# OliBomby/Mapperatorinator

Hardware: NVIDIA H100
Metric: event tokens/sec end-to-end (mel+T5+DiT) (higher is better)
Workload: dtype f32

## Files before the change

### mapperatorinator_b200/csrc/engine_dit.cu

```cuda
#include <algorithm>
#include <cmath>
#include <cstring>
#include <map>
#include <tuple>
#include <unordered_map>
#include <vector>

#include "../../include/mapperatorinator_b200.h"
#include "common.cuh"
#include "kernels.h"

using namespace mb200;

namespace {

struct DevBufD {
    void* p = nullptr; size_t bytes = 0;
    int ensure(size_t need) {
        if (need <= bytes) return 0;
        if (p) cudaFree(p);
        p = nullptr; bytes = 0;
        MB_CUDA_CHECK(cudaMalloc(&p, need));
        bytes = need;
        return 0;
// ... 224 lines not shown
    dd->t0_w = W("t_embedder.mlp.0.weight"); dd->t0_b = W("t_embedder.mlp.0.bias"); dd->t2_w = W("t_embedder.mlp.2.weight"); dd->t2_b = W("t_embedder.mlp.2.bias");
    dd->y0_w = W("y_embedder.class_embedding.0.weight"); dd->y0_b = W("y_embedder.class_embedding.0.bias");
    dd->y2_w = W("y_embedder.class_embedding.2.weight"); dd->y2_b = W("y_embedder.class_embedding.2.bias");
    dd->fada_w = W("final_layer.adaLN_modulation.1.weight"); dd->fada_b = W("final_layer.adaLN_modulation.1.bias");
    dd->flin_w = W("final_layer.linear.weight"); dd->flin_b = W("final_layer.linear.bias");
    for (int i = 0; i < c.depth; ++i) {
        const std::string p = "blocks." + std::to_string(i) + ".";
        dd->blocks.push_back(BlockW{W(p + "attn.in_proj_weight"), W(p + "attn.in_proj_bias"), W(p + "attn.out_proj.weight"), W(p + "attn.out_proj.bias"),
                                    W(p + "mlp.fc1.weight"), W(p + "mlp.fc1.bias"), W(p + "mlp.fc2.weight"), W(p + "mlp.fc2.bias"),
                                    W(p + "adaLN_modulation.1.weight"), W(p + "adaLN_modulation.1.bias")});
    }
    {
        int dev = 0;
        cudaGetDevice(&dev);
        cudaDeviceGetAttribute(&dd->gemm.num_sms, cudaDevAttrMultiProcessorCount, dev);
    }
    for (const auto& n : names)
        if (n.find("weight") != std::string::npos && sizes.at(n) >= (size_t)64 * 32) MB_TRY(dd->gemm.register_weight(W(n), (long long)sizes.at(n)));
    MB_CUDA_CHECK(cudaDeviceSynchronize());
    dd->pos_freqs = W("__pos_freqs"); dd->t_freqs = W("__t_freqs");
    MB_REQUIRE(dd->host_w.at("context_embedder.mlp.0.weight").size() == (size_t)d * (c.in_channels * c.pos_freq_dim + c.context_size),
               "context_embedder shape mismatch");
    {
        const size_t R = (size_t)std::max(2, c.max_batch) * c.max_seq_len;
        const size_t K0 = (size_t)c.in_channels * c.pos_freq_dim + c.context_size;
        MB_TRY(dd->gemm.reserve((size_t)64 << 20, R * std::max((size_t)d * c.mlp_ratio, K0) * 8 + 1024));
        dd->gemm.frozen = true;
        MB_TRY(dd->attn.reserve(attn_tc_workspace_bytes(std::max(2, c.max_batch), c.heads, c.max_seq_len, c.max_seq_len)));
        dd->attn.frozen = true;
    }
    dd->host_w.clear();
    dd->finalized = true;
    return 0;
}

namespace {

GemmParams gb(const float* A, long long lda, const float* W, long long ldw, float* C, long long ldc, const float* bias, int M, int N, int K) {
    GemmParams g{};
    g.A = plain_map(A, lda); g.W = W; g.ldw = ldw; g.C = plain_map(C, ldc); g.bias = bias; g.act = ACT_NONE; g.alpha = 1.f;
    g.gate = nullptr; g.gate_ld = 0; g.gate_rpb = 1; g.R = RowMap{nullptr, 0, 0, 0}; g.M = M; g.N = N; g.K = K;
    return g;
}

int ln_mod(const float* x, float* y, const float* shift, const float* scale, long long mod_ld, int T, int rows, int d, cudaStream_t st) {
    LayerNormParams p{};
    p.x = x; p.ldx = d; p.y = y; p.ldy = d; p.weight = nullptr; p.bias = nullptr; p.shift = shift; p.scale = scale; p.mod_ld = mod_ld;
    p.rows_per_batch = T; p.rows = rows; p.dim = d; p.eps = 1e-6f;
    return launch_layernorm(p, st);
// ... 280 lines not shown
```

### mapperatorinator_b200/csrc/engine_model.cu

```cuda
#include <algorithm>
#include <cstring>
#include <functional>
#include <map>
#include <tuple>
#include <unordered_map>
#include <vector>

#include "../../include/mapperatorinator_b200.h"
#include "common.cuh"
#include "kernels.h"

using namespace mb200;

namespace {

struct DevBuf {
    void* p = nullptr;
    size_t bytes = 0;
    int ensure(size_t need, bool zero = false) {
        if (need <= bytes) return 0;
        if (p) cudaFree(p);
        p = nullptr; bytes = 0;
        MB_CUDA_CHECK(cudaMalloc(&p, need));
        bytes = need;
// ... 258 lines not shown
        if (cross) {
            l.ln2_w = base + o.v[6]; l.ln2_b = base + o.v[7]; l.wq_c = base + o.v[8]; l.bq_c = base + o.v[9];
            l.wkv_c = base + o.v[10]; l.bkv_c = base + o.v[11]; l.wo_c = base + o.v[12]; l.bo_c = base + o.v[13];
        }
        l.ln3_w = base + o.v[14]; l.ln3_b = base + o.v[15]; l.fc1_w = base + o.v[16]; l.fc1_b = base + o.v[17];
        l.fc2_w = base + o.v[18]; l.fc2_b = base + o.v[19];
        return l;
    };
    for (auto& o : eo) m->enc.push_back(fill(o, false));
    for (auto& o : dof) m->dec.push_back(fill(o, true));
    m->host_w.clear();
    {
        const long long dd = (long long)d * d;
        auto reg = [&](const float* w, long long n) -> int { return m->gemm.register_weight(w, n); };
        MB_TRY(reg(m->emb_w, (long long)d * c.mel.n_mels));
        MB_TRY(reg(m->conv1_w, 3 * dd)); MB_TRY(reg(m->conv2_w, 3 * dd));
        for (const auto& l : m->enc) {
            MB_TRY(reg(l.wqkv, 3 * dd)); MB_TRY(reg(l.wo, dd));
            MB_TRY(reg(l.fc1_w, (long long)f * d)); MB_TRY(reg(l.fc2_w, (long long)f * d));
        }
        for (const auto& l : m->dec) MB_TRY(reg(l.wkv_c, 2 * dd));
        MB_CUDA_CHECK(cudaDeviceSynchronize());
        const size_t chunk = (size_t)std::min(std::max(1, c.max_windows), 16);
        const size_t a_floats = std::max({chunk * (size_t)(c.src_seq_len / 2) * f, chunk * (size_t)(c.src_seq_len + 2) * d,
                                          chunk * (size_t)c.src_seq_len * c.mel.n_mels});
        m->gemm.num_sms = std::max(1, m->num_sms_phys);
        MB_TRY(m->gemm.reserve((size_t)64 << 20, a_floats * 8 + 1024));
        m->gemm.frozen = true;
        MB_TRY(m->attn.reserve(attn_tc_workspace_bytes((int)chunk, c.heads, c.src_seq_len / 2, c.src_seq_len / 2)));
        m->attn.frozen = true;
    }

    m->max_rows = std::max(1, c.max_batch);
    MB_TRY(m->cross_kv.ensure((size_t)c.decoder_layers * m->cross_layer_stride() * sizeof(float)));
    MB_TRY(m->self_kv.ensure((size_t)c.decoder_layers * m->self_layer_stride() * sizeof(float)));
    MB_TRY(m->g_state.ensure(sizeof(GenState) + (size_t)m->max_rows * sizeof(RowState)));
    MB_TRY(m->g_cfg.ensure((size_t)m->max_rows * sizeof(SampleConfig)));
    MB_TRY(m->g_vflags.ensure((size_t)m->max_rows * c.vocab_size_in));
    MB_TRY(m->g_ids.ensure((size_t)m->max_rows * c.tgt_seq_len * sizeof(long long)));
    MB_TRY(m->g_prefill_ids.ensure((size_t)m->max_rows * c.tgt_seq_len * sizeof(long long)));
    MB_TRY(m->g_keyvalid.ensure((size_t)m->max_rows * c.tgt_seq_len));
    MB_TRY(m->g_leftpad.ensure(m->max_rows * sizeof(int)));
    MB_TRY(m->g_rowslot.ensure((size_t)3 * m->max_rows * sizeof(int)));
    MB_TRY(m->g_finished.ensure(m->max_rows));
    {
        const size_t tgt = (size_t)m->max_rows * c.tgt_seq_len;
        m->h_stage_bytes = tgt * 8 * 2 + tgt + (size_t)2 * m->max_rows * 4 + c.vocab_size_in + sizeof(GenState) + sizeof(SampleConfig) + 8 * 16;
        MB_CUDA_CHECK(cudaMallocHost(&m->h_stage, m->h_stage_bytes));
        MB_CUDA_CHECK(cudaEventCreateWithFlags(&m->stage_ev, cudaEventDisableTiming));
    }
// ... 1160 lines not shown
```

### mapperatorinator_b200/csrc/gemm.cu

```cuda
#include <algorithm>
#include <cstdlib>
#include "common.cuh"
#include "kernels.h"

namespace mb200 {

namespace {

constexpr int BM = 128, BN = 128, BK = 16, PAD = 4;

template <int MH>
__global__ void __launch_bounds__(256, 2) gemm_f32_kernel(GemmParams p) {
    constexpr int TM = 64 * MH;
    __shared__ __align__(16) float As[2][BK][TM + PAD];
    __shared__ __align__(16) float Bs[2][BK][BN + PAD];

    const int tid = threadIdx.x;
    const int tx = tid & 15, ty = tid >> 4;
    const long long m0 = (long long)blockIdx.y * TM;
    const int n0 = blockIdx.x * BN;

    const int lrow = tid >> 2;
    const int lk = (tid & 3) * 4;
    const float* a_ptr[2];
// ... 100 lines not shown
                if (rrow) v += rrow[nn];
                crow[nn] = v;
            }
        }
    }
}

__global__ void __launch_bounds__(256) gemm_splitk_reduce_kernel(GemmParams p) {
    const long long idx = (long long)blockIdx.x * 256 + threadIdx.x;
    if (idx >= (long long)p.M * p.N) return;
    const long long m = idx / p.N;
    const int n = (int)(idx - m * p.N);
    float v = p.splitk_ws[m * p.N + n];
    for (int z = 1; z < p.splitk; ++z) v += p.splitk_ws[((long long)z * p.M + m) * p.N + n];
    if (p.bias) v += __ldg(p.bias + n);
    v = apply_act(v, p.act) * p.alpha;
    if (p.gate) v *= __ldg(p.gate + ((p.m_base + m) / p.gate_rpb) * p.gate_ld + n);
    if (p.R.ptr) v += p.R.row(p.m_base + m)[n];
    p.C.row(p.m_base + m)[n] = v;
}

}

int GemmCtx::reserve(size_t splitk_need, size_t a_split_need) {
    auto grow = [&](float*& ptr, size_t& have, size_t need) -> int {
        if (need <= have) return 0;
        MB_REQUIRE(!frozen, "GEMM scratch is referenced by a captured CUDA graph and cannot grow (reserve the largest shape before capturing)");
        if (ptr) MB_CUDA_CHECK(cudaFree(ptr));
        ptr = nullptr; have = 0;
        MB_CUDA_CHECK(cudaMalloc(&ptr, need));
        have = need;
        return 0;
    };
    int s = grow(splitk_ws, splitk_bytes, splitk_need);
    if (s) return s;
    s = grow(a_split, a_split_bytes, a_split_need);
    if (s) return s;
    if (!tc_err) { MB_CUDA_CHECK(cudaMalloc(&tc_err, 4)); MB_CUDA_CHECK(cudaMemset(tc_err, 0, 4)); }
    return 0;
}

int GemmCtx::error() {
    if (!tc_err) return 0;
    int h = 0;
    cudaMemcpy(&h, tc_err, 4, cudaMemcpyDeviceToHost);
    return h;
}

void GemmCtx::destroy() {
    for (auto& kv : mirrors) cudaFree(const_cast<float*>(kv.second.hi));
    mirrors.clear();
    if (splitk_ws) cudaFree(splitk_ws);
    if (a_split) cudaFree(a_split);
    if (tc_err) cudaFree(tc_err);
    splitk_ws = a_split = nullptr; tc_err = nullptr; splitk_bytes = a_split_bytes = 0; frozen = false;
}

GemmCtx* default_gemm_ctx() {
    static GemmCtx ctx;
    static bool init = false;
    if (!init) {
        int dev = 0;
        cudaGetDevice(&dev);
        cudaDeviceGetAttribute(&ctx.num_sms, cudaDevAttrMultiProcessorCount, dev);
        init = true;
    }
    return &ctx;
}

int gemm_splits_simt(int N, int K, int num_sms, int* k_per_split) {
    const int tiles_n = (N + BN - 1) / BN;
    int splits = 1;
    if (tiles_n * 2 <= num_sms && K >= 64) splits = std::max(1, std::min((num_sms + tiles_n - 1) / tiles_n, K / 32));
    const int kps = ((K + splits - 1) / splits + BK - 1) / BK * BK;
    splits = (K + kps - 1) / kps;
    *k_per_split = kps;
    return splits;
}
// ... 8 lines not shown
int launch_gemm(const GemmParams& p, cudaStream_t stream, GemmCtx* ctx) {
    MB_REQUIRE(ctx != nullptr, "GEMM needs its engine's scratch context");
    MB_REQUIRE(p.K % 4 == 0, "GEMM K must be a multiple of 4 (float4 loads)");
    MB_REQUIRE(p.A.ld % 4 == 0 && p.ldw % 4 == 0, "GEMM operand row strides must be multiples of 4 floats");
    MB_REQUIRE((reinterpret_cast<uintptr_t>(p.A.ptr) & 15) == 0 && (reinterpret_cast<uintptr_t>(p.W) & 15) == 0,
               "GEMM operands must be 16-byte aligned");
    if (p.M <= 0 || p.N <= 0) return 0;
    if (tc_gemm_eligible(p, ctx)) return launch_gemm_tc(p, stream, ctx);
    int kps = 0;
    const int splits = gemm_splits_simt(p.N, p.K, ctx->num_sms, &kps);
    const int tiles_n = (p.N + BN - 1) / BN;
    const bool half = p.M <= BM;
    const int tm = half ? BM / 2 : BM;
    if (splits == 1) {
        dim3 grid(tiles_n, (unsigned)((p.M + tm - 1) / tm));
        if (half) gemm_f32_kernel<1><<<grid, 256, 0, stream>>>(p);
        else gemm_f32_kernel<2><<<grid, 256, 0, stream>>>(p);
        MB_LAUNCH_CHECK();
        ++g_launch_count;
        return 0;
    }
    const size_t row_bytes = (size_t)splits * p.N * sizeof(float);
    if (row_bytes * (size_t)p.M > ctx->splitk_bytes && !ctx->frozen) {
        const int s = ctx->reserve(std::max(row_bytes * (size_t)std::min(p.M, 2048), (size_t)64 << 20), 0);
        if (s) return s;
    }
    MB_REQUIRE(ctx->splitk_bytes >= row_bytes * BM, "split-K workspace smaller than one row tile");
    const long long rows_per_pass = std::min<long long>(p.M, (long long)(ctx->splitk_bytes / row_bytes) / BM * BM);
    for (long long m0 = 0; m0 < p.M; m0 += rows_per_pass) {
        GemmParams q = p;
        q.m_base = p.m_base + m0;
        q.M = (int)std::min<long long>(rows_per_pass, p.M - m0);
        q.splitk_ws = ctx->splitk_ws; q.splitk = splits; q.k_per_split = kps; q.split_mode = 1;
        const dim3 grid(tiles_n, (unsigned)((q.M + tm - 1) / tm), splits);
        if (half) gemm_f32_kernel<1><<<grid, 256, 0, stream>>>(q);
        else gemm_f32_kernel<2><<<grid, 256, 0, stream>>>(q);
        MB_LAUNCH_CHECK();
        ++g_launch_count;
        const int s = launch_splitk_reduce(q, stream);
        if (s) return s;
    }
    return 0;
}

}
```

### mapperatorinator_b200/csrc/gemm_tc.cu

```cuda
#include <cuda.h>
#include <algorithm>
#include <cmath>
#include <cstdio>
#include <cstdlib>
#include <vector>
#include <map>
#include <tuple>
#include <unordered_map>

#include "common.cuh"
#include "kernels.h"
#include "wgmma.cuh"

namespace mb200 {

int g_tc_enabled = 1;

namespace {

constexpr int TC_BM = 128, TC_BN = 128, TC_BK = 32, TC_STAGES = 3, TC_THREADS = 384, TC_CONSUMERS = 256;
constexpr int TC_TILE_BYTES = TC_BM * TC_BK * 4;
constexpr int TC_STAGE_BYTES = 4 * TC_TILE_BYTES;
constexpr int TC_EPI_LD = TC_BN + 8;
static_assert(TC_BM * TC_EPI_LD * 4 <= TC_STAGES * TC_STAGE_BYTES, "epilogue staging fits the pipeline stages");

struct TcBarriers {
    unsigned long long full[TC_STAGES];
    unsigned long long empty[TC_STAGES];
};

__device__ __forceinline__ unsigned s32(const void* p) { return (unsigned)__cvta_generic_to_shared(p); }

__device__ __forceinline__ bool bar_wait(unsigned long long* bar, unsigned parity, int* err) {
    for (long long spin = 0; spin < (1ll << 22); ++spin) {
        unsigned ok;
        asm volatile("{ .reg .pred p; mbarrier.try_wait.parity.shared::cta.b64 p, [%1], %2; selp.u32 %0, 1, 0, p; }"
                     : "=r"(ok) : "r"(s32(bar)), "r"(parity) : "memory");
        if (ok) return true;
    }
    atomicExch(err, 3);
    return false;
}

__global__ void __launch_bounds__(TC_THREADS, 1)
gemm_tf32x3_kernel(const __grid_constant__ CUtensorMap map_a, const __grid_constant__ CUtensorMap map_alo,
                   const __grid_constant__ CUtensorMap map_w, const __grid_constant__ CUtensorMap map_wlo, GemmParams p, int a_rpb, int* err) {
    extern __shared__ unsigned char tc_smem_raw[];
    unsigned char* smem = reinterpret_cast<unsigned char*>((reinterpret_cast<uintptr_t>(tc_smem_raw) + 1023) & ~uintptr_t(1023));
    TcBarriers* bars = reinterpret_cast<TcBarriers*>(smem + TC_STAGES * TC_STAGE_BYTES);
    const int tid = threadIdx.x;
    const int n0 = blockIdx.x * TC_BN;
    const long long m0 = (long long)blockIdx.y * TC_BM;
    const int nkb_all = (p.K + TC_BK - 1) / TC_BK;
    const int kpb = p.splitk > 1 ? p.k_per_split / TC_BK : nkb_all;
    const bool grid_split = p.split_mode == 1, tile_split = p.split_mode == 2;
    const int kb0 = grid_split ? blockIdx.z * kpb : 0;
    const int nkb = grid_split ? max(0, min(nkb_all - kb0, kpb)) : nkb_all;

    if (tid == 0) {
        for (int s = 0; s < TC_STAGES; ++s) {
            asm volatile("mbarrier.init.shared::cta.b64 [%0], 1;" ::"r"(s32(&bars->full[s])));
            asm volatile("mbarrier.init.shared::cta.b64 [%0], %1;" ::"r"(s32(&bars->empty[s])), "r"(TC_CONSUMERS));
        }
        asm volatile("fence.mbarrier_init.release.cluster;" ::: "memory");
    }
    __syncthreads();

    if (tid < 128) {
        asm volatile("setmaxnreg.dec.sync.aligned.u32 40;");
        if (tid == 0) {
            const int a_b = a_rpb > 0 ? (int)(m0 / a_rpb) : 0;
            const int a_t = a_rpb > 0 ? (int)(m0 - (long long)a_b * a_rpb) : (int)m0;
            for (int kb = 0; kb < nkb; ++kb) {
                const int s = kb % TC_STAGES;
                const unsigned ph = (kb / TC_STAGES) & 1;
                if (!bar_wait(&bars->empty[s], ph ^ 1, err)) break;
                unsigned char* st = smem + s * TC_STAGE_BYTES;
                const unsigned fb = s32(&bars->full[s]);
                asm volatile("{ .reg .b64 t; mbarrier.arrive.expect_tx.shared::cta.b64 t, [%0], %1; }" ::"r"(fb), "r"(TC_STAGE_BYTES) : "memory");
                const int k0 = (kb0 + kb) * TC_BK;
                asm volatile("cp.async.bulk.tensor.3d.shared::cluster.global.mbarrier::complete_tx::bytes [%0], [%1, {%2, %3, %4}], [%5];"
                             ::"r"(s32(st)), "l"(&map_a), "r"(k0), "r"(a_t), "r"(a_b), "r"(fb) : "memory");
                asm volatile("cp.async.bulk.tensor.3d.shared::cluster.global.mbarrier::complete_tx::bytes [%0], [%1, {%2, %3, %4}], [%5];"
                             ::"r"(s32(st + TC_TILE_BYTES)), "l"(&map_alo), "r"(k0), "r"(a_t), "r"(a_b), "r"(fb) : "memory");
                asm volatile("cp.async.bulk.tensor.2d.shared::cluster.global.mbarrier::complete_tx::bytes [%0], [%1, {%2, %3}], [%4];"
                             ::"r"(s32(st + 2 * TC_TILE_BYTES)), "l"(&map_w), "r"(k0), "r"(n0), "r"(fb) : "memory");
                asm volatile("cp.async.bulk.tensor.2d.shared::cluster.global.mbarrier::complete_tx::bytes [%0], [%1, {%2, %3}], [%4];"
                             ::"r"(s32(st + 3 * TC_TILE_BYTES)), "l"(&map_wlo), "r"(k0), "r"(n0), "r"(fb) : "memory");
            }
        }
        return;
    }

    asm volatile("setmaxnreg.inc.sync.aligned.u32 232;");
    const int ct = tid - 128;
    const int cg = ct >> 7;
    float acc[64], sum[64];
#pragma unroll
    for (int i = 0; i < 64; ++i) { acc[i] = 0.f; sum[i] = 0.f; }
#pragma unroll 1
    for (int kb = 0; kb < nkb; ++kb) {
        const int s = kb % TC_STAGES;
        const unsigned ph = (kb / TC_STAGES) & 1;
        if (!bar_wait(&bars->full[s], ph, err)) break;
        const unsigned base = s32(smem + s * TC_STAGE_BYTES);
        const unsigned a_off = (unsigned)cg * (64 * 128);
        const int z = tile_split ? kb / kpb : 0, kr = tile_split ? kb - z * kpb : kb;
        gmma_fence_regs(acc);
        gmma_fence();
#pragma unroll
        for (int sub = 0; sub < TC_BK / 8; ++sub) {
            const unsigned off = sub * 32;
            const unsigned long long a_hi = gmma_desc(base + a_off + off), a_lo = gmma_desc(base + TC_TILE_BYTES + a_off + off);
            const unsigned long long w_hi = gmma_desc(base + 2 * TC_TILE_BYTES + off), w_lo = gmma_desc(base + 3 * TC_TILE_BYTES + off);
            gmma_m64n128k8_ss(acc, a_hi, w_hi, (kr > 0 || sub > 0) ? 1u : 0u);
            gmma_m64n128k8_ss(acc, a_hi, w_lo, 1u);
            gmma_m64n128k8_ss(acc, a_lo, w_hi, 1u);
        }
        gmma_commit();
        gmma_wait<0>();
        gmma_fence_regs(acc);
        asm volatile("{ .reg .b64 t; mbarrier.arrive.shared::cta.b64 t, [%0]; }" ::"r"(s32(&bars->empty[s])) : "memory");
        if (kb == nkb - 1 || (tile_split && kr == kpb - 1)) {
            if (z == 0) {
#pragma unroll
                for (int i = 0; i < 64; ++i) sum[i] = acc[i];
            } else {
#pragma unroll
                for (int i = 0; i < 64; ++i) sum[i] += acc[i];
            }
        }
    }

    asm volatile("bar.sync 1, %0;" ::"n"(TC_CONSUMERS) : "memory");
    float* stg = reinterpret_cast<float*>(smem);
    {
        const int w = (ct >> 5) & 3, lane = ct & 31, gid = lane >> 2, tig = lane & 3;
        const int r = cg * 64 + w * 16 + gid;
#pragma unroll
        for (int j = 0; j < 16; ++j) {
            const int c = 8 * j + 2 * tig;
            *reinterpret_cast<float2*>(stg + r * TC_EPI_LD + c) = make_float2(sum[4 * j], sum[4 * j + 1]);
            *reinterpret_cast<float2*>(stg + (r + 8) * TC_EPI_LD + c) = make_float2(sum[4 * j + 2], sum[4 * j + 3]);
        }
    }
    asm volatile("bar.sync 1, %0;" ::"n"(TC_CONSUMERS) : "memory");
    const int lane = ct & 31, cw = ct >> 5;
    const bool has_r = !grid_split && p.R.ptr != nullptr, has_g = !grid_split && p.gate != nullptr;
    float bias_v[TC_BN / 32];
#pragma unroll
    for (int c = 0; c < TC_BN / 32; ++c) {
        const int n = n0 + 32 * c + lane;
        bias_v[c] = (!grid_split && p.bias && n < p.N) ? __ldg(p.bias + n) : 0.f;
    }
#pragma unroll 1
    for (int rr = 0; rr < 16; ++rr) {
        const int row = cw * 16 + rr;
        const long long m = m0 + row;
        if (m >= p.M) break;
        float* crow = grid_split ? p.splitk_ws + ((long long)blockIdx.z * p.M + m) * p.N : p.C.row(m);
        const float* rrow = has_r ? p.R.row(m) : nullptr;
        const float* grow = has_g ? p.gate + (m / p.gate_rpb) * p.gate_ld : nullptr;
#pragma unroll
        for (int c = 0; c < TC_BN / 32; ++c) {
            const int n = n0 + 32 * c + lane;
            if (n >= p.N) continue;
            float x = stg[row * TC_EPI_LD + 32 * c + lane];
            if (!grid_split) {
                if (p.bias) x += bias_v[c];
                x = apply_act(x, p.act) * p.alpha;
                if (has_g) x *= __ldg(grow + n);
                if (has_r) x += rrow[n];
            }
            crow[n] = x;
        }
    }
}

__device__ __forceinline__ float rn_tf32(float x) {
    unsigned u;
    asm("cvt.rna.tf32.f32 %0, %1;" : "=r"(u) : "f"(x));
    return __uint_as_float(u);
}
__global__ void tf32_split_kernel(const float* __restrict__ x, float* __restrict__ hi, float* __restrict__ lo, long long n4) {
    const long long i = (long long)blockIdx.x * blockDim.x + threadIdx.x;
    if (i >= n4) return;
    const float4 v = reinterpret_cast<const float4*>(x)[i];
    float4 h, l;
    h.x = rn_tf32(v.x); h.y = rn_tf32(v.y); h.z = rn_tf32(v.z); h.w = rn_tf32(v.w);
    l.x = rn_tf32(v.x - h.x); l.y = rn_tf32(v.y - h.y); l.z = rn_tf32(v.z - h.z); l.w = rn_tf32(v.w - h.w);
    reinterpret_cast<float4*>(hi)[i] = h;
    reinterpret_cast<float4*>(lo)[i] = l;
}

typedef CUresult (*EncodeTiledFn)(CUtensorMap*, CUtensorMapDataType, cuuint32_t, void*, const cuuint64_t*, const cuuint64_t*, const cuuint32_t*,
                                  const cuuint32_t*, CUtensorMapInterleave, CUtensorMapSwizzle, CUtensorMapL2promotion, CUtensorMapFloatOOBfill);

EncodeTiledFn encode_fn() {
    static EncodeTiledFn fn = nullptr;
    if (!fn) {
        void* p = nullptr;
        cudaDriverEntryPointQueryResult q;
        if (cudaGetDriverEntryPoint("cuTensorMapEncodeTiled", &p, cudaEnableDefault, &q) == cudaSuccess && q == cudaDriverEntryPointSuccess)
            fn = reinterpret_cast<EncodeTiledFn>(p);
    }
    return fn;
// ... 10 lines not shown
    CUresult r = fn(out, CU_TENSOR_MAP_DATA_TYPE_FLOAT32, (cuuint32_t)rank, const_cast<float*>(base), dims, strides, box, estr,
                    CU_TENSOR_MAP_INTERLEAVE_NONE, CU_TENSOR_MAP_SWIZZLE_128B, CU_TENSOR_MAP_L2_PROMOTION_L2_128B, CU_TENSOR_MAP_FLOAT_OOB_FILL_NONE);
    MB_REQUIRE(r == CUDA_SUCCESS, "cuTensorMapEncodeTiled failed (" + std::to_string((int)r) + ")");
    return 0;
}

}

int gemm_splits_tc(int N, int K, int num_sms, int* k_per_split) {
    const int tiles_ref = 4 * ((N + TC_BN - 1) / TC_BN), nkb = (K + TC_BK - 1) / TC_BK;
    int splits = std::max(1, std::min({4, num_sms / std::max(1, tiles_ref), nkb / 8}));
    const int kpb = (nkb + splits - 1) / splits;
    splits = (nkb + kpb - 1) / kpb;
    *k_per_split = kpb * TC_BK;
    return splits;
}

static int g_tc_tested = 0;
static void tc_self_test() {
    g_tc_tested = 1;
    GemmCtx ctx;
    ctx.num_sms = default_gemm_ctx()->num_sms;
    bool all_ok = true;
    const int shapes[3][3] = {{512, 128, 96}, {512, 128, 1024}, {2048, 256, 1024}};
    for (int t = 0; t < 3 && all_ok; ++t) {
        const int M = shapes[t][0], N = shapes[t][1], K = shapes[t][2];
        std::vector<float> a((size_t)M * K), w((size_t)N * K), c((size_t)M * N);
        unsigned s = 12345u + t;
        auto rnd = [&]() { s = s * 1664525u + 1013904223u; return (float)((s >> 8) & 0xFFFF) / 32768.0f - 1.0f; };
        for (auto& v : a) v = rnd();
        for (auto& v : w) v = rnd();
        float *da = nullptr, *dw = nullptr, *dc = nullptr;
        bool ok = cudaMalloc(&da, a.size() * 4) == cudaSuccess && cudaMalloc(&dw, w.size() * 4) == cudaSuccess && cudaMalloc(&dc, c.size() * 4) == cudaSuccess;
        if (ok) {
            cudaMemcpy(da, a.data(), a.size() * 4, cudaMemcpyHostToDevice);
            cudaMemcpy(dw, w.data(), w.size() * 4, cudaMemcpyHostToDevice);
            GemmParams g{};
            g.A = plain_map(da, K); g.W = dw; g.ldw = K; g.C = plain_map(dc, N); g.alpha = 1.f; g.gate_rpb = 1; g.M = M; g.N = N; g.K = K;
            ok = ctx.register_weight(dw, (long long)N * K) == 0 && launch_gemm_tc(g, nullptr, &ctx) == 0 && cudaDeviceSynchronize() == cudaSuccess &&
                 ctx.error() == 0;
            if (ok) {
                cudaMemcpy(c.data(), dc, c.size() * 4, cudaMemcpyDeviceToHost);
                double worst = 0;
                for (int m = 0; m < M; m += 37)
                    for (int n = 0; n < N; n += 5) {
                        double r = 0;
                        for (int k = 0; k < K; ++k) r += (double)a[(size_t)m * K + k] * (double)w[(size_t)n * K + k];
// ... 10 lines not shown
    ctx.destroy();
    if (!all_ok) {
        g_tc_enabled = 0;
        fprintf(stderr, "[mapperatorinator_b200] WARNING: wgmma GEMM self-test FAILED — tensor-core path disabled, using the fp32 SIMT GEMM\n");
        cudaGetLastError();
    }
}

bool tc_gemm_eligible(const GemmParams& p, GemmCtx* ctx) {
    if (g_tc_enabled && !g_tc_tested) tc_self_test();
    if (!g_tc_enabled || p.m_base != 0) return false;
    if (p.M < 512 || p.N < 64 || p.K < 32 || p.K % 4 != 0) return false;
    if (ctx->mirrors.find(p.W) == ctx->mirrors.end()) return false;
    if (p.A.rpb != 0 && (p.A.rpb % TC_BM) != 0) return false;
    if ((reinterpret_cast<uintptr_t>(p.A.ptr) & 15) || (reinterpret_cast<uintptr_t>(p.W) & 15) || (p.A.ld % 4) || (p.ldw % 4)) return false;
    if (p.A.rpb != 0 && (p.A.bstride % 4)) return false;
    return true;
}

int launch_gemm_tc(const GemmParams& p, cudaStream_t stream, GemmCtx* ctx) {
    const Tf32Mirror wm = ctx->mirrors.at(p.W);
    const long long batches = p.A.rpb ? (p.M + p.A.rpb - 1) / p.A.rpb : 1;
    const long long rpb = p.A.rpb ? p.A.rpb : p.M;
    const long long extent = (batches - 1) * (p.A.rpb ? p.A.bstride : 0) + (rpb - 1) * p.A.ld + p.K;
    const long long n4 = (extent + 3) / 4;
    dim3 grid((p.N + TC_BN - 1) / TC_BN, (unsigned)((p.M + TC_BM - 1) / TC_BM));
    GemmParams q = p;
    q.splitk = gemm_splits_tc(p.N, p.K, ctx->num_sms, &q.k_per_split);
    q.split_mode = 0; q.splitk_ws = nullptr;
    if (q.splitk > 1) {
        const int tiles = (int)(grid.x * grid.y);
        q.split_mode = tiles * 4 <= ctx->num_sms * 3 ? 1 : 2;
    } else {
        q.splitk = 1;
    }
    {
        const int s = ctx->reserve(q.split_mode == 1 ? (size_t)q.splitk * p.M * p.N * sizeof(float) : 0, (size_t)n4 * 32);
        if (s) return s;
    }
    if (q.split_mode == 1) { q.splitk_ws = ctx->splitk_ws; grid.z = q.splitk; }
    float* a_hi = ctx->a_split;
    float* a_lo = ctx->a_split + n4 * 4;
    tf32_split_kernel<<<(unsigned)((n4 + 255) / 256), 256, 0, stream>>>(p.A.ptr, a_hi, a_lo, n4);
    MB_LAUNCH_CHECK();
    CUtensorMap ma, mal, mw, mwl;
    MB_REQUIRE(make_map(&ma, a_hi, p.K, rpb, p.A.ld, batches, p.A.rpb ? p.A.bstride : 0, 3) == 0, "tensor map Ahi");
    MB_REQUIRE(make_map(&mal, a_lo, p.K, rpb, p.A.ld, batches, p.A.rpb ? p.A.bstride : 0, 3) == 0, "tensor map Alo");
    MB_REQUIRE(make_map(&mw, wm.hi, p.K, p.N, p.ldw, 1, 0, 2) == 0, "tensor map Whi");
    MB_REQUIRE(make_map(&mwl, wm.lo, p.K, p.N, p.ldw, 1, 0, 2) == 0, "tensor map Wlo");
    static bool configured = false;
    const int smem = TC_STAGES * TC_STAGE_BYTES + (int)sizeof(TcBarriers) + 1024;
    if (!configured) {
        MB_CUDA_CHECK(cudaFuncSetAttribute(gemm_tf32x3_kernel, cudaFuncAttributeMaxDynamicSharedMemorySize, smem));
        configured = true;
    }
    gemm_tf32x3_kernel<<<grid, TC_THREADS, smem, stream>>>(ma, mal, mw, mwl, q, p.A.rpb, ctx->tc_err);
    MB_LAUNCH_CHECK();
    g_launch_count += 2;
    if (q.split_mode == 1) return launch_splitk_reduce(q, stream);
    return 0;
}

void GemmCtx::unregister_weight(const float* w) {
    auto it = mirrors.find(w);
    if (it == mirrors.end()) return;
    cudaFree(const_cast<float*>(it->second.hi));
    mirrors.erase(it);
}

int GemmCtx::register_weight(const float* w, long long numel) {
    unregister_weight(w);
    float* buf = nullptr;
    const long long n4 = (numel + 3) / 4;
    MB_CUDA_CHECK(cudaMalloc(&buf, (size_t)n4 * 32));
    tf32_split_kernel<<<(unsigned)((n4 + 255) / 256), 256>>>(w, buf, buf + n4 * 4, n4);
    MB_LAUNCH_CHECK();
    mirrors[w] = Tf32Mirror{buf, buf + n4 * 4};
    return 0;
}

}
// ... 1 lines not shown
```

### mapperatorinator_b200/csrc/kernels.h

```cpp
#pragma once
#include <unordered_map>
#include "common.cuh"

namespace mb200 {

struct GemmParams {
    RowMap A;
    const float* W;
    long long ldw;
    RowMap C;
    const float* bias;
    int act;
    float alpha;
    const float* gate;
    long long gate_ld;
    int gate_rpb;
    RowMap R;
    int M, N, K;
    float* splitk_ws; int splitk; int k_per_split; int split_mode;
    long long m_base;
};

struct Tf32Mirror { const float* hi; const float* lo; };
struct GemmCtx {
    int num_sms = 132;
    float* splitk_ws = nullptr; size_t splitk_bytes = 0;
    float* a_split = nullptr; size_t a_split_bytes = 0;
    int* tc_err = nullptr;
    bool frozen = false;
    std::unordered_map<const float*, Tf32Mirror> mirrors;
    int reserve(size_t splitk_need, size_t a_split_need);
    int register_weight(const float* w, long long numel);
    void unregister_weight(const float* w);
    int error();
    void destroy();
};
GemmCtx* default_gemm_ctx();
int launch_gemm(const GemmParams& p, cudaStream_t stream, GemmCtx* ctx);
extern int g_tc_enabled;
int launch_splitk_reduce(const GemmParams& q, cudaStream_t stream);
bool tc_gemm_eligible(const GemmParams& p, GemmCtx* ctx);
int launch_gemm_tc(const GemmParams& p, cudaStream_t stream, GemmCtx* ctx);
int gemm_splits_tc(int N, int K, int num_sms, int* k_per_split);
int gemm_splits_simt(int N, int K, int num_sms, int* k_per_split);

struct LayerNormParams {
    const float* x; long long ldx;
    float* y; long long ldy;
    const float* weight; const float* bias;
    const float* shift; const float* scale; long long mod_ld; int rows_per_batch;
    int rows, dim;
    float eps;
};
int launch_layernorm(const LayerNormParams& p, cudaStream_t stream);
// ... 261 lines not shown
```

### mapperatorinator_b200/csrc/wgmma.cuh

```cuda
#pragma once
#include <cuda_runtime.h>

namespace mb200 {

__device__ __forceinline__ unsigned long long gmma_desc(unsigned smem_addr) {
    unsigned long long d = 0;
    d |= (unsigned long long)((smem_addr & 0x3FFFF) >> 4);
    d |= (unsigned long long)1 << 16;
    d |= (unsigned long long)(1024 >> 4) << 32;
    d |= (unsigned long long)1 << 62;
    return d;
}

__device__ __forceinline__ void gmma_fence() { asm volatile("wgmma.fence.sync.aligned;" ::: "memory"); }
__device__ __forceinline__ void gmma_commit() { asm volatile("wgmma.commit_group.sync.aligned;" ::: "memory"); }
template <int N>
__device__ __forceinline__ void gmma_wait() { asm volatile("wgmma.wait_group.sync.aligned %0;" ::"n"(N) : "memory"); }

template <int R>
__device__ __forceinline__ void gmma_fence_regs(float (&d)[R]) {
#pragma unroll
    for (int i = 0; i < R; ++i) asm volatile("" : "+f"(d[i])::"memory");
}

__device__ __forceinline__ void gmma_m64n128k8_ss(float (&d)[64], unsigned long long da, unsigned long long db, unsigned scale_d) {
    asm volatile(
        "{ .reg .pred p; setp.ne.b32 p, %66, 0; wgmma.mma_async.sync.aligned.m64n128k8.f32.tf32.tf32 {%0, %1, %2, %3, %4, %5, %6, %7, %8, "
        "%9, %10, %11, %12, %13, %14, %15, %16, %17, %18, %19, %20, %21, %22, %23, %24, %25, %26, %27, %28, %29, %30, %31, %32, %33, %34, "
        "%35, %36, %37, %38, %39, %40, %41, %42, %43, %44, %45, %46, %47, %48, %49, %50, %51, %52, %53, %54, %55, %56, %57, %58, %59, %60, "
        "%61, %62, %63}, %64, %65, p, 1, 1; }"
        : "+f"(d[0]), "+f"(d[1]), "+f"(d[2]), "+f"(d[3]), "+f"(d[4]), "+f"(d[5]), "+f"(d[6]), "+f"(d[7]), "+f"(d[8]), "+f"(d[9]),
          "+f"(d[10]), "+f"(d[11]), "+f"(d[12]), "+f"(d[13]), "+f"(d[14]), "+f"(d[15]), "+f"(d[16]), "+f"(d[17]), "+f"(d[18]),
          "+f"(d[19]), "+f"(d[20]), "+f"(d[21]), "+f"(d[22]), "+f"(d[23]), "+f"(d[24]), "+f"(d[25]), "+f"(d[26]), "+f"(d[27]),
          "+f"(d[28]), "+f"(d[29]), "+f"(d[30]), "+f"(d[31]), "+f"(d[32]), "+f"(d[33]), "+f"(d[34]), "+f"(d[35]), "+f"(d[36]),
          "+f"(d[37]), "+f"(d[38]), "+f"(d[39]), "+f"(d[40]), "+f"(d[41]), "+f"(d[42]), "+f"(d[43]), "+f"(d[44]), "+f"(d[45]),
          "+f"(d[46]), "+f"(d[47]), "+f"(d[48]), "+f"(d[49]), "+f"(d[50]), "+f"(d[51]), "+f"(d[52]), "+f"(d[53]), "+f"(d[54]),
          "+f"(d[55]), "+f"(d[56]), "+f"(d[57]), "+f"(d[58]), "+f"(d[59]), "+f"(d[60]), "+f"(d[61]), "+f"(d[62]), "+f"(d[63])
        : "l"(da), "l"(db), "r"(scale_d));
}

__device__ __forceinline__ void gmma_m64n64k8_ss(float (&d)[32], unsigned long long da, unsigned long long db, unsigned scale_d) {
    asm volatile(
        "{ .reg .pred p; setp.ne.b32 p, %34, 0; wgmma.mma_async.sync.aligned.m64n64k8.f32.tf32.tf32 {%0, %1, %2, %3, %4, %5, %6, %7, %8, "
        "%9, %10, %11, %12, %13, %14, %15, %16, %17, %18, %19, %20, %21, %22, %23, %24, %25, %26, %27, %28, %29, %30, %31}, %32, %33, p, 1, 1; }"
        : "+f"(d[0]), "+f"(d[1]), "+f"(d[2]), "+f"(d[3]), "+f"(d[4]), "+f"(d[5]), "+f"(d[6]), "+f"(d[7]), "+f"(d[8]), "+f"(d[9]),
          "+f"(d[10]), "+f"(d[11]), "+f"(d[12]), "+f"(d[13]), "+f"(d[14]), "+f"(d[15]), "+f"(d[16]), "+f"(d[17]), "+f"(d[18]),
          "+f"(d[19]), "+f"(d[20]), "+f"(d[21]), "+f"(d[22]), "+f"(d[23]), "+f"(d[24]), "+f"(d[25]), "+f"(d[26]), "+f"(d[27]),
          "+f"(d[28]), "+f"(d[29]), "+f"(d[30]), "+f"(d[31])
        : "l"(da), "l"(db), "r"(scale_d));
}

__device__ __forceinline__ void gmma_m64n64k8_rs(float (&d)[32], const unsigned (&a)[4], unsigned long long db, unsigned scale_d) {
    asm volatile(
        "{ .reg .pred p; setp.ne.b32 p, %37, 0; wgmma.mma_async.sync.aligned.m64n64k8.f32.tf32.tf32 {%0, %1, %2, %3, %4, %5, %6, %7, %8, "
        "%9, %10, %11, %12, %13, %14, %15, %16, %17, %18, %19, %20, %21, %22, %23, %24, %25, %26, %27, %28, %29, %30, %31}, "
        "{%32, %33, %34, %35}, %36, p, 1, 1; }"
        : "+f"(d[0]), "+f"(d[1]), "+f"(d[2]), "+f"(d[3]), "+f"(d[4]), "+f"(d[5]), "+f"(d[6]), "+f"(d[7]), "+f"(d[8]), "+f"(d[9]),
          "+f"(d[10]), "+f"(d[11]), "+f"(d[12]), "+f"(d[13]), "+f"(d[14]), "+f"(d[15]), "+f"(d[16]), "+f"(d[17]), "+f"(d[18]),
          "+f"(d[19]), "+f"(d[20]), "+f"(d[21]), "+f"(d[22]), "+f"(d[23]), "+f"(d[24]), "+f"(d[25]), "+f"(d[26]), "+f"(d[27]),
          "+f"(d[28]), "+f"(d[29]), "+f"(d[30]), "+f"(d[31])
        : "r"(a[0]), "r"(a[1]), "r"(a[2]), "r"(a[3]), "l"(db), "r"(scale_d));
}

// ... 2 lines not shown
```

Baseline: 1871.

## Fuse activation TF32 hi/lo split into wgmma GEMM via register-sourced A operands

Removes the separate tf32_split_kernel and its scratch buffer. The GEMM now loads raw fp32 A tiles via TMA, reads them with ldmatrix, splits them into hi/lo TF32 in registers, and feeds register-sourced wgmma. This frees a stage's worth of smem, so the pipeline goes from 3 to 4 stages. Stage release is also deferred so wgmma overlaps the next sub-tile, split-K mode selection now uses wave rounds, and the gated/residual epilogue prefetches rows. The cost is more register pressure and per-consumer conversion work, plus riskier async ordering.

Result: faster. 1912 (median of 6 runs) (+2.2%).

```diff
diff --git a/mapperatorinator_b200/csrc/engine_dit.cu b/mapperatorinator_b200/csrc/engine_dit.cu
--- a/mapperatorinator_b200/csrc/engine_dit.cu
+++ b/mapperatorinator_b200/csrc/engine_dit.cu
@@ -270,9 +270,7 @@
     MB_REQUIRE(dd->host_w.at("context_embedder.mlp.0.weight").size() == (size_t)d * (c.in_channels * c.pos_freq_dim + c.context_size),
                "context_embedder shape mismatch");
     {
-        const size_t R = (size_t)std::max(2, c.max_batch) * c.max_seq_len;
-        const size_t K0 = (size_t)c.in_channels * c.pos_freq_dim + c.context_size;
-        MB_TRY(dd->gemm.reserve((size_t)64 << 20, R * std::max((size_t)d * c.mlp_ratio, K0) * 8 + 1024));
+        MB_TRY(dd->gemm.reserve((size_t)64 << 20));
         dd->gemm.frozen = true;
         MB_TRY(dd->attn.reserve(attn_tc_workspace_bytes(std::max(2, c.max_batch), c.heads, c.max_seq_len, c.max_seq_len)));
         dd->attn.frozen = true;
diff --git a/mapperatorinator_b200/csrc/engine_model.cu b/mapperatorinator_b200/csrc/engine_model.cu
--- a/mapperatorinator_b200/csrc/engine_model.cu
+++ b/mapperatorinator_b200/csrc/engine_model.cu
@@ -304,10 +304,8 @@
         for (const auto& l : m->dec) MB_TRY(reg(l.wkv_c, 2 * dd));
         MB_CUDA_CHECK(cudaDeviceSynchronize());
         const size_t chunk = (size_t)std::min(std::max(1, c.max_windows), 16);
-        const size_t a_floats = std::max({chunk * (size_t)(c.src_seq_len / 2) * f, chunk * (size_t)(c.src_seq_len + 2) * d,
-                                          chunk * (size_t)c.src_seq_len * c.mel.n_mels});
         m->gemm.num_sms = std::max(1, m->num_sms_phys);
-        MB_TRY(m->gemm.reserve((size_t)64 << 20, a_floats * 8 + 1024));
+        MB_TRY(m->gemm.reserve((size_t)64 << 20));
         m->gemm.frozen = true;
         MB_TRY(m->attn.reserve(attn_tc_workspace_bytes((int)chunk, c.heads, c.src_seq_len / 2, c.src_seq_len / 2)));
         m->attn.frozen = true;
diff --git a/mapperatorinator_b200/csrc/gemm.cu b/mapperatorinator_b200/csrc/gemm.cu
--- a/mapperatorinator_b200/csrc/gemm.cu
+++ b/mapperatorinator_b200/csrc/gemm.cu
@@ -146,7 +146,7 @@
 
 }
 
-int GemmCtx::reserve(size_t splitk_need, size_t a_split_need) {
+int GemmCtx::reserve(size_t splitk_need) {
     auto grow = [&](float*& ptr, size_t& have, size_t need) -> int {
         if (need <= have) return 0;
         MB_REQUIRE(!frozen, "GEMM scratch is referenced by a captured CUDA graph and cannot grow (reserve the largest shape before capturing)");
@@ -156,9 +156,7 @@
         have = need;
         return 0;
     };
-    int s = grow(splitk_ws, splitk_bytes, splitk_need);
-    if (s) return s;
-    s = grow(a_split, a_split_bytes, a_split_need);
+    const int s = grow(splitk_ws, splitk_bytes, splitk_need);
     if (s) return s;
     if (!tc_err) { MB_CUDA_CHECK(cudaMalloc(&tc_err, 4)); MB_CUDA_CHECK(cudaMemset(tc_err, 0, 4)); }
     return 0;
@@ -175,9 +173,8 @@
     for (auto& kv : mirrors) cudaFree(const_cast<float*>(kv.second.hi));
     mirrors.clear();
     if (splitk_ws) cudaFree(splitk_ws);
-    if (a_split) cudaFree(a_split);
     if (tc_err) cudaFree(tc_err);
-    splitk_ws = a_split = nullptr; tc_err = nullptr; splitk_bytes = a_split_bytes = 0; frozen = false;
+    splitk_ws = nullptr; tc_err = nullptr; splitk_bytes = 0; frozen = false;
 }
 
 GemmCtx* default_gemm_ctx() {
@@ -232,7 +229,7 @@
     }
     const size_t row_bytes = (size_t)splits * p.N * sizeof(float);
     if (row_bytes * (size_t)p.M > ctx->splitk_bytes && !ctx->frozen) {
-        const int s = ctx->reserve(std::max(row_bytes * (size_t)std::min(p.M, 2048), (size_t)64 << 20), 0);
+        const int s = ctx->reserve(std::max(row_bytes * (size_t)std::min(p.M, 2048), (size_t)64 << 20));
         if (s) return s;
     }
     MB_REQUIRE(ctx->splitk_bytes >= row_bytes * BM, "split-K workspace smaller than one row tile");
diff --git a/mapperatorinator_b200/csrc/gemm_tc.cu b/mapperatorinator_b200/csrc/gemm_tc.cu
--- a/mapperatorinator_b200/csrc/gemm_tc.cu
+++ b/mapperatorinator_b200/csrc/gemm_tc.cu
@@ -18,9 +18,9 @@
 
 namespace {
 
-constexpr int TC_BM = 128, TC_BN = 128, TC_BK = 32, TC_STAGES = 3, TC_THREADS = 384, TC_CONSUMERS = 256;
+constexpr int TC_BM = 128, TC_BN = 128, TC_BK = 32, TC_STAGES = 4, TC_THREADS = 384, TC_CONSUMERS = 256;
 constexpr int TC_TILE_BYTES = TC_BM * TC_BK * 4;
-constexpr int TC_STAGE_BYTES = 4 * TC_TILE_BYTES;
+constexpr int TC_STAGE_BYTES = 3 * TC_TILE_BYTES;
 constexpr int TC_EPI_LD = TC_BN + 8;
 static_assert(TC_BM * TC_EPI_LD * 4 <= TC_STAGES * TC_STAGE_BYTES, "epilogue staging fits the pipeline stages");
 
@@ -42,9 +42,20 @@
     return false;
 }
 
+__device__ __forceinline__ float rn_tf32(float x) {
+    unsigned u;
+    asm("cvt.rna.tf32.f32 %0, %1;" : "=r"(u) : "f"(x));
+    return __uint_as_float(u);
+}
+
+__device__ __forceinline__ void ldsm_x4(unsigned (&r)[4], unsigned addr) {
+    asm volatile("ldmatrix.sync.aligned.m8n8.x4.shared.b16 {%0, %1, %2, %3}, [%4];"
+                 : "=r"(r[0]), "=r"(r[1]), "=r"(r[2]), "=r"(r[3]) : "r"(addr) : "memory");
+}
+
 __global__ void __launch_bounds__(TC_THREADS, 1)
-gemm_tf32x3_kernel(const __grid_constant__ CUtensorMap map_a, const __grid_constant__ CUtensorMap map_alo,
-                   const __grid_constant__ CUtensorMap map_w, const __grid_constant__ CUtensorMap map_wlo, GemmParams p, int a_rpb, int* err) {
+gemm_tf32x3_kernel(const __grid_constant__ CUtensorMap map_a, const __grid_constant__ CUtensorMap map_w, const __grid_constant__ CUtensorMap map_wlo,
+                   GemmParams p, int a_rpb, int* err) {
     extern __shared__ unsigned char tc_smem_raw[];
     unsigned char* smem = reinterpret_cast<unsigned char*>((reinterpret_cast<uintptr_t>(tc_smem_raw) + 1023) & ~uintptr_t(1023));
     TcBarriers* bars = reinterpret_cast<TcBarriers*>(smem + TC_STAGES * TC_STAGE_BYTES);
@@ -81,12 +92,10 @@
                 const int k0 = (kb0 + kb) * TC_BK;
                 asm volatile("cp.async.bulk.tensor.3d.shared::cluster.global.mbarrier::complete_tx::bytes [%0], [%1, {%2, %3, %4}], [%5];"
                              ::"r"(s32(st)), "l"(&map_a), "r"(k0), "r"(a_t), "r"(a_b), "r"(fb) : "memory");
-                asm volatile("cp.async.bulk.tensor.3d.shared::cluster.global.mbarrier::complete_tx::bytes [%0], [%1, {%2, %3, %4}], [%5];"
-                             ::"r"(s32(st + TC_TILE_BYTES)), "l"(&map_alo), "r"(k0), "r"(a_t), "r"(a_b), "r"(fb) : "memory");
                 asm volatile("cp.async.bulk.tensor.2d.shared::cluster.global.mbarrier::complete_tx::bytes [%0], [%1, {%2, %3}], [%4];"
-                             ::"r"(s32(st + 2 * TC_TILE_BYTES)), "l"(&map_w), "r"(k0), "r"(n0), "r"(fb) : "memory");
+                             ::"r"(s32(st + TC_TILE_BYTES)), "l"(&map_w), "r"(k0), "r"(n0), "r"(fb) : "memory");
                 asm volatile("cp.async.bulk.tensor.2d.shared::cluster.global.mbarrier::complete_tx::bytes [%0], [%1, {%2, %3}], [%4];"
-                             ::"r"(s32(st + 3 * TC_TILE_BYTES)), "l"(&map_wlo), "r"(k0), "r"(n0), "r"(fb) : "memory");
+                             ::"r"(s32(st + 2 * TC_TILE_BYTES)), "l"(&map_wlo), "r"(k0), "r"(n0), "r"(fb) : "memory");
             }
         }
         return;
@@ -98,30 +107,46 @@
     float acc[64], sum[64];
 #pragma unroll
     for (int i = 0; i < 64; ++i) { acc[i] = 0.f; sum[i] = 0.f; }
+    const int lane = ct & 31, lj = lane >> 3, li = lane & 7;
+    const unsigned a_row = (unsigned)(cg * 64 + ((ct >> 5) & 3) * 16 + (lj & 1) * 8 + li) * 128;
+    unsigned slot_hi[2][4], slot_lo[2][4];
+    int pending = -1;
 #pragma unroll 1
     for (int kb = 0; kb < nkb; ++kb) {
         const int s = kb % TC_STAGES;
         const unsigned ph = (kb / TC_STAGES) & 1;
         if (!bar_wait(&bars->full[s], ph, err)) break;
         const unsigned base = s32(smem + s * TC_STAGE_BYTES);
-        const unsigned a_off = (unsigned)cg * (64 * 128);
         const int z = tile_split ? kb / kpb : 0, kr = tile_split ? kb - z * kpb : kb;
-        gmma_fence_regs(acc);
-        gmma_fence();
+        if (kr == 0) gmma_fence_regs(acc);
 #pragma unroll
         for (int sub = 0; sub < TC_BK / 8; ++sub) {
+            unsigned raw[4];
+            ldsm_x4(raw, base + a_row + ((unsigned)((2 * sub + (lj >> 1)) ^ li) << 4));
+            unsigned (&ahi)[4] = slot_hi[sub & 1], (&alo)[4] = slot_lo[sub & 1];
+            gmma_wait<1>();
+            if (sub == 1 && pending >= 0) {
+                asm volatile("{ .reg .b64 t; mbarrier.arrive.shared::cta.b64 t, [%0]; }" ::"r"(s32(&bars->empty[pending])) : "memory");
+                pending = -1;
+            }
+#pragma unroll
+            for (int u = 0; u < 4; ++u) {
+                const float x = __uint_as_float(raw[u]), hi = rn_tf32(x);
+                ahi[u] = __float_as_uint(hi);
+                alo[u] = __float_as_uint(rn_tf32(x - hi));
+            }
+            gmma_fence();
             const unsigned off = sub * 32;
-            const unsigned long long a_hi = gmma_desc(base + a_off + off), a_lo = gmma_desc(base + TC_TILE_BYTES + a_off + off);
-            const unsigned long long w_hi = gmma_desc(base + 2 * TC_TILE_BYTES + off), w_lo = gmma_desc(base + 3 * TC_TILE_BYTES + off);
-            gmma_m64n128k8_ss(acc, a_hi, w_hi, (kr > 0 || sub > 0) ? 1u : 0u);
-            gmma_m64n128k8_ss(acc, a_hi, w_lo, 1u);
-            gmma_m64n128k8_ss(acc, a_lo, w_hi, 1u);
-        }
-        gmma_commit();
-        gmma_wait<0>();
-        gmma_fence_regs(acc);
-        asm volatile("{ .reg .b64 t; mbarrier.arrive.shared::cta.b64 t, [%0]; }" ::"r"(s32(&bars->empty[s])) : "memory");
+            const unsigned long long w_hi = gmma_desc(base + TC_TILE_BYTES + off), w_lo = gmma_desc(base + 2 * TC_TILE_BYTES + off);
+            gmma_m64n128k8_rs(acc, ahi, w_hi, (kr > 0 || sub > 0) ? 1u : 0u);
+            gmma_m64n128k8_rs(acc, ahi, w_lo, 1u);
+            gmma_m64n128k8_rs(acc, alo, w_hi, 1u);
+            gmma_commit();
+        }
         if (kb == nkb - 1 || (tile_split && kr == kpb - 1)) {
+            gmma_wait<0>();
+            gmma_fence_regs(acc);
+            asm volatile("{ .reg .b64 t; mbarrier.arrive.shared::cta.b64 t, [%0]; }" ::"r"(s32(&bars->empty[s])) : "memory");
             if (z == 0) {
 #pragma unroll
                 for (int i = 0; i < 64; ++i) sum[i] = acc[i];
@@ -129,13 +154,17 @@
 #pragma unroll
                 for (int i = 0; i < 64; ++i) sum[i] += acc[i];
             }
-        }
-    }
+        } else {
+            pending = s;
+        }
+    }
+    gmma_wait<0>();
+    gmma_fence_regs(acc);
 
     asm volatile("bar.sync 1, %0;" ::"n"(TC_CONSUMERS) : "memory");
     float* stg = reinterpret_cast<float*>(smem);
     {
-        const int w = (ct >> 5) & 3, lane = ct & 31, gid = lane >> 2, tig = lane & 3;
+        const int w = (ct >> 5) & 3, gid = lane >> 2, tig = lane & 3;
         const int r = cg * 64 + w * 16 + gid;
 #pragma unroll
         for (int j = 0; j < 16; ++j) {
@@ -145,7 +174,7 @@
         }
     }
     asm volatile("bar.sync 1, %0;" ::"n"(TC_CONSUMERS) : "memory");
-    const int lane = ct & 31, cw = ct >> 5;
+    const int cw = ct >> 5;
     const bool has_r = !grid_split && p.R.ptr != nullptr, has_g = !grid_split && p.gate != nullptr;
     float bias_v[TC_BN / 32];
 #pragma unroll
@@ -153,35 +182,65 @@
         const int n = n0 + 32 * c + lane;
         bias_v[c] = (!grid_split && p.bias && n < p.N) ? __ldg(p.bias + n) : 0.f;
     }
+    if (!has_r && !has_g) {
 #pragma unroll 1
-    for (int rr = 0; rr < 16; ++rr) {
-        const int row = cw * 16 + rr;
-        const long long m = m0 + row;
-        if (m >= p.M) break;
-        float* crow = grid_split ? p.splitk_ws + ((long long)blockIdx.z * p.M + m) * p.N : p.C.row(m);
-        const float* rrow = has_r ? p.R.row(m) : nullptr;
-        const float* grow = has_g ? p.gate + (m / p.gate_rpb) * p.gate_ld : nullptr;
-#pragma unroll
-        for (int c = 0; c < TC_BN / 32; ++c) {
-            const int n = n0 + 32 * c + lane;
-            if (n >= p.N) continue;
-            float x = stg[row * TC_EPI_LD + 32 * c + lane];
-            if (!grid_split) {
+        for (int rr = 0; rr < 16; ++rr) {
+            const int row = cw * 16 + rr;
+            const long long m = m0 + row;
+            if (m >= p.M) break;
+            float* crow = grid_split ? p.splitk_ws + ((long long)blockIdx.z * p.M + m) * p.N : p.C.row(m);
+#pragma unroll
+            for (int c = 0; c < TC_BN / 32; ++c) {
+                const int n = n0 + 32 * c + lane;
+                if (n >= p.N) continue;
+                float x = stg[row * TC_EPI_LD + 32 * c + lane];
+                if (!grid_split) {
+                    if (p.bias) x += bias_v[c];
+                    x = apply_act(x, p.act) * p.alpha;
+                }
+                crow[n] = x;
+            }
+        }
+        return;
+    }
+    constexpr int EPI_ROWS = 4;
+#pragma unroll 1
+    for (int r0 = 0; r0 < 16; r0 += EPI_ROWS) {
+        float gv[EPI_ROWS][TC_BN / 32], rv[EPI_ROWS][TC_BN / 32];
+#pragma unroll
+        for (int j = 0; j < EPI_ROWS; ++j) {
+            const long long m = m0 + cw * 16 + r0 + j;
+            const float* rrow = has_r && m < p.M ? p.R.row(m) : nullptr;
+            const float* grow = has_g && m < p.M ? p.gate + (m / p.gate_rpb) * p.gate_ld : nullptr;
+#pragma unroll
+            for (int c = 0; c < TC_BN / 32; ++c) {
+                const int n = n0 + 32 * c + lane;
+                gv[j][c] = grow && n < p.N ? __ldg(grow + n) : 1.f;
+                rv[j][c] = rrow && n < p.N ? rrow[n] : 0.f;
+            }
+        }
+#pragma unroll
+        for (int j = 0; j < EPI_ROWS; ++j) {
+            const int row = cw * 16 + r0 + j;
+            const long long m = m0 + row;
+            if (m >= p.M) break;
+            float* crow = p.C.row(m);
+#pragma unroll
+            for (int c = 0; c < TC_BN / 32; ++c) {
+                const int n = n0 + 32 * c + lane;
+                if (n >= p.N) continue;
+                float x = stg[row * TC_EPI_LD + 32 * c + lane];
                 if (p.bias) x += bias_v[c];
                 x = apply_act(x, p.act) * p.alpha;
-                if (has_g) x *= __ldg(grow + n);
-                if (has_r) x += rrow[n];
-            }
-            crow[n] = x;
-        }
-    }
-}
-
-__device__ __forceinline__ float rn_tf32(float x) {
-    unsigned u;
-    asm("cvt.rna.tf32.f32 %0, %1;" : "=r"(u) : "f"(x));
-    return __uint_as_float(u);
-}
+                if (has_g) x *= gv[j][c];
+                if (has_r) x += rv[j][c];
+                crow[n] = x;
+            }
+        }
+        if (m0 + cw * 16 + r0 + EPI_ROWS >= p.M) break;
+    }
+}
+
 __global__ void tf32_split_kernel(const float* __restrict__ x, float* __restrict__ hi, float* __restrict__ lo, long long n4) {
     const long long i = (long long)blockIdx.x * blockDim.x + threadIdx.x;
     if (i >= n4) return;
@@ -238,7 +297,7 @@
     GemmCtx ctx;
     ctx.num_sms = default_gemm_ctx()->num_sms;
     bool all_ok = true;
-    const int shapes[3][3] = {{512, 128, 96}, {512, 128, 1024}, {2048, 256, 1024}};
+    const int shapes[3][3] = {{512, 128, 96}, {512, 128, 1024}, {4096, 512, 1024}};
     for (int t = 0; t < 3 && all_ok; ++t) {
         const int M = shapes[t][0], N = shapes[t][1], K = shapes[t][2];
         std::vector<float> a((size_t)M * K), w((size_t)N * K), c((size_t)M * N);
@@ -295,30 +354,24 @@
     const Tf32Mirror wm = ctx->mirrors.at(p.W);
     const long long batches = p.A.rpb ? (p.M + p.A.rpb - 1) / p.A.rpb : 1;
     const long long rpb = p.A.rpb ? p.A.rpb : p.M;
-    const long long extent = (batches - 1) * (p.A.rpb ? p.A.bstride : 0) + (rpb - 1) * p.A.ld + p.K;
-    const long long n4 = (extent + 3) / 4;
     dim3 grid((p.N + TC_BN - 1) / TC_BN, (unsigned)((p.M + TC_BM - 1) / TC_BM));
     GemmParams q = p;
     q.splitk = gemm_splits_tc(p.N, p.K, ctx->num_sms, &q.k_per_split);
     q.split_mode = 0; q.splitk_ws = nullptr;
     if (q.splitk > 1) {
-        const int tiles = (int)(grid.x * grid.y);
-        q.split_mode = tiles * 4 <= ctx->num_sms * 3 ? 1 : 2;
+        const int tiles = (int)(grid.x * grid.y), sms = std::max(1, ctx->num_sms);
+        const int grid_rounds = (tiles * q.splitk + sms - 1) / sms, tile_rounds = q.splitk * ((tiles + sms - 1) / sms);
+        q.split_mode = grid_rounds < tile_rounds ? 1 : 2;
     } else {
         q.splitk = 1;
     }
     {
-        const int s = ctx->reserve(q.split_mode == 1 ? (size_t)q.splitk * p.M * p.N * sizeof(float) : 0, (size_t)n4 * 32);
+        const int s = ctx->reserve(q.split_mode == 1 ? (size_t)q.splitk * p.M * p.N * sizeof(float) : 0);
         if (s) return s;
     }
     if (q.split_mode == 1) { q.splitk_ws = ctx->splitk_ws; grid.z = q.splitk; }
-    float* a_hi = ctx->a_split;
-    float* a_lo = ctx->a_split + n4 * 4;
-    tf32_split_kernel<<<(unsigned)((n4 + 255) / 256), 256, 0, stream>>>(p.A.ptr, a_hi, a_lo, n4);
-    MB_LAUNCH_CHECK();
-    CUtensorMap ma, mal, mw, mwl;
-    MB_REQUIRE(make_map(&ma, a_hi, p.K, rpb, p.A.ld, batches, p.A.rpb ? p.A.bstride : 0, 3) == 0, "tensor map Ahi");
-    MB_REQUIRE(make_map(&mal, a_lo, p.K, rpb, p.A.ld, batches, p.A.rpb ? p.A.bstride : 0, 3) == 0, "tensor map Alo");
+    CUtensorMap ma, mw, mwl;
+    MB_REQUIRE(make_map(&ma, p.A.ptr, p.K, rpb, p.A.ld, batches, p.A.rpb ? p.A.bstride : 0, 3) == 0, "tensor map A");
     MB_REQUIRE(make_map(&mw, wm.hi, p.K, p.N, p.ldw, 1, 0, 2) == 0, "tensor map Whi");
     MB_REQUIRE(make_map(&mwl, wm.lo, p.K, p.N, p.ldw, 1, 0, 2) == 0, "tensor map Wlo");
     static bool configured = false;
@@ -327,9 +380,9 @@
         MB_CUDA_CHECK(cudaFuncSetAttribute(gemm_tf32x3_kernel, cudaFuncAttributeMaxDynamicSharedMemorySize, smem));
         configured = true;
     }
-    gemm_tf32x3_kernel<<<grid, TC_THREADS, smem, stream>>>(ma, mal, mw, mwl, q, p.A.rpb, ctx->tc_err);
+    gemm_tf32x3_kernel<<<grid, TC_THREADS, smem, stream>>>(ma, mw, mwl, q, p.A.rpb, ctx->tc_err);
     MB_LAUNCH_CHECK();
-    g_launch_count += 2;
+    ++g_launch_count;
     if (q.split_mode == 1) return launch_splitk_reduce(q, stream);
     return 0;
 }
diff --git a/mapperatorinator_b200/csrc/kernels.h b/mapperatorinator_b200/csrc/kernels.h
--- a/mapperatorinator_b200/csrc/kernels.h
+++ b/mapperatorinator_b200/csrc/kernels.h
@@ -25,11 +25,10 @@
 struct GemmCtx {
     int num_sms = 132;
     float* splitk_ws = nullptr; size_t splitk_bytes = 0;
-    float* a_split = nullptr; size_t a_split_bytes = 0;
     int* tc_err = nullptr;
     bool frozen = false;
     std::unordered_map<const float*, Tf32Mirror> mirrors;
-    int reserve(size_t splitk_need, size_t a_split_need);
+    int reserve(size_t splitk_need);
     int register_weight(const float* w, long long numel);
     void unregister_weight(const float* w);
     int error();
diff --git a/mapperatorinator_b200/csrc/wgmma.cuh b/mapperatorinator_b200/csrc/wgmma.cuh
--- a/mapperatorinator_b200/csrc/wgmma.cuh
+++ b/mapperatorinator_b200/csrc/wgmma.cuh
@@ -39,6 +39,22 @@
         : "l"(da), "l"(db), "r"(scale_d));
 }
 
+__device__ __forceinline__ void gmma_m64n128k8_rs(float (&d)[64], const unsigned (&a)[4], unsigned long long db, unsigned scale_d) {
+    asm volatile(
+        "{ .reg .pred p; setp.ne.b32 p, %69, 0; wgmma.mma_async.sync.aligned.m64n128k8.f32.tf32.tf32 {%0, %1, %2, %3, %4, %5, %6, %7, %8, "
+        "%9, %10, %11, %12, %13, %14, %15, %16, %17, %18, %19, %20, %21, %22, %23, %24, %25, %26, %27, %28, %29, %30, %31, %32, %33, %34, "
+        "%35, %36, %37, %38, %39, %40, %41, %42, %43, %44, %45, %46, %47, %48, %49, %50, %51, %52, %53, %54, %55, %56, %57, %58, %59, %60, "
+        "%61, %62, %63}, {%64, %65, %66, %67}, %68, p, 1, 1; }"
+        : "+f"(d[0]), "+f"(d[1]), "+f"(d[2]), "+f"(d[3]), "+f"(d[4]), "+f"(d[5]), "+f"(d[6]), "+f"(d[7]), "+f"(d[8]), "+f"(d[9]),
+          "+f"(d[10]), "+f"(d[11]), "+f"(d[12]), "+f"(d[13]), "+f"(d[14]), "+f"(d[15]), "+f"(d[16]), "+f"(d[17]), "+f"(d[18]),
+          "+f"(d[19]), "+f"(d[20]), "+f"(d[21]), "+f"(d[22]), "+f"(d[23]), "+f"(d[24]), "+f"(d[25]), "+f"(d[26]), "+f"(d[27]),
+          "+f"(d[28]), "+f"(d[29]), "+f"(d[30]), "+f"(d[31]), "+f"(d[32]), "+f"(d[33]), "+f"(d[34]), "+f"(d[35]), "+f"(d[36]),
+          "+f"(d[37]), "+f"(d[38]), "+f"(d[39]), "+f"(d[40]), "+f"(d[41]), "+f"(d[42]), "+f"(d[43]), "+f"(d[44]), "+f"(d[45]),
+          "+f"(d[46]), "+f"(d[47]), "+f"(d[48]), "+f"(d[49]), "+f"(d[50]), "+f"(d[51]), "+f"(d[52]), "+f"(d[53]), "+f"(d[54]),
+          "+f"(d[55]), "+f"(d[56]), "+f"(d[57]), "+f"(d[58]), "+f"(d[59]), "+f"(d[60]), "+f"(d[61]), "+f"(d[62]), "+f"(d[63])
+        : "r"(a[0]), "r"(a[1]), "r"(a[2]), "r"(a[3]), "l"(db), "r"(scale_d));
+}
+
 __device__ __forceinline__ void gmma_m64n64k8_ss(float (&d)[32], unsigned long long da, unsigned long long db, unsigned scale_d) {
     asm volatile(
         "{ .reg .pred p; setp.ne.b32 p, %34, 0; wgmma.mma_async.sync.aligned.m64n64k8.f32.tf32.tf32 {%0, %1, %2, %3, %4, %5, %6, %7, %8, "
```
